# aluo7/ViT-SOM

Measured on AMD Instinct MI355X. Metric: images/sec/node ViT-SOM 40x40 CIFAR-10 bs512 (training step: fwd+bwd+all-reduce+AdamW), higher is better.
Workload: dtype f32 (Linear GEMMs on bf16 MFMA: forward from an exact 3xbf16 operand split, six products; weight / input gradients from a 2xbf16 split, three products, rel. error 4e-6)

## Files before the change

### include/vitsom_hip.h

```cpp
#ifndef VITSOM_HIP_H
#define VITSOM_HIP_H

#include <stddef.h>
#include <stdint.h>

#ifdef __cplusplus
extern "C" {
#endif

typedef struct ihipStream_t* vsom_stream_t;

#define VSOM_OK 0
#define VSOM_EINVAL (-1)
#define VSOM_EALIGN (-2)
#define VSOM_EUNSUPPORTED (-3)
#define VSOM_EWORKSPACE (-4)

#define VSOM_VERSION 100

#define VSOM_DIST_COSINE 0
#define VSOM_DIST_EUCLIDEAN 1
#define VSOM_DIST_MANHATTAN 2

int vsom_version(void);
const char* vsom_last_error_string(void);

int vsom_linear_fwd(const float* X, long ldx, const float* W, const float* bias, float* Y, long ldy,
                    int M, int N, int K, vsom_stream_t stream);

int vsom_linear_gelu_fwd(const float* X, long ldx, const float* W, const float* bias, float* Ygrad,
                         float* Yact, int M, int N, int K, vsom_stream_t stream);

int vsom_linear_relu_fwd(const float* X, long ldx, const float* W, const float* bias, float* Ygrad,
                         float* Yact, int M, int N, int K, vsom_stream_t stream);

int vsom_linear_residual_fwd(const float* X, long ldx, const float* W, const float* bias,
                             const float* R, long ldr, int r_mod, float* Y, long ldy, int M, int N,
                             int K, vsom_stream_t stream);

int vsom_linear_bwd_input(const float* dY, long lddy, const float* W, float* dX, long lddx, int M,
                          int N, int K, int accumulate, const float* gelu_grad, vsom_stream_t stream);

int vsom_linear_bwd_input_t(const float* dY, long lddy, const float* Wt, float* dX, long lddx, int M,
                            int N, int K, int accumulate, const float* gelu_grad, vsom_stream_t stream);

int vsom_transpose_many(const float* src_base, float* dst_base, const long long* table, int count,
                        int max_rows, int max_cols, vsom_stream_t stream);

#define VSOM_GEMM_F32 0
#define VSOM_GEMM_SPLIT_BF16 1
#define VSOM_GEMM_SPLIT_BF16_GRAD3 2
int vsom_set_gemm_mode(int mode);
int vsom_get_gemm_mode(void);

size_t vsom_linear_bwd_weight_workspace_bytes(int M, int N, int K);
int vsom_linear_bwd_weight(const float* dY, long lddy, const float* X, long ldx, float* dW, float* db,
                           int M, int N, int K, void* ws, size_t ws_bytes, vsom_stream_t stream);

int vsom_patch_embed_fwd(const float* img, const float* Wpe, const float* bpe, const float* pos,
                         const float* cls_token, float* tokens, float* xp_ws, int B, int C, int S,
                         int p, int E, vsom_stream_t stream);
size_t vsom_patch_embed_bwd_workspace_bytes(int B, int C, int S, int p, int E);
int vsom_patch_embed_bwd(const float* dtokens, const float* xp_ws, float* dWpe, float* dbpe,
                         float* dcls_token, int B, int C, int S, int p, int E, void* ws,
                         size_t ws_bytes, vsom_stream_t stream);

int vsom_layernorm_fwd(const float* X, const float* gamma, const float* beta, float* Y, float* mean,
                       float* rstd, int rows, int cols, float eps, vsom_stream_t stream);
size_t vsom_layernorm_bwd_workspace_bytes(int rows, int cols);
int vsom_layernorm_bwd(const float* dY, const float* X, const float* mean, const float* rstd,
                       const float* gamma, const float* resid, float* dX, float* dgamma, float* dbeta,
                       int rows, int cols, void* ws, size_t ws_bytes, vsom_stream_t stream);
#define VSOM_LN_JOB_WORDS 4
int vsom_layernorm_bwd_deferrable(int rows, int cols);
int vsom_layernorm_bwd_partial(const float* dY, const float* X, const float* mean, const float* rstd,
                               const float* gamma, const float* resid, float* dX, int rows, int cols, void* part,
                               size_t part_bytes, vsom_stream_t stream);
int vsom_layernorm_bwd_finish_many(const int64_t* jobs_dev, int first, int count, int max_cols, vsom_stream_t stream);

int vsom_linear_bwd_input_ln_supported(int M, int N, int K);
size_t vsom_linear_bwd_input_ln_partial_bytes(int M, int K);
int vsom_linear_bwd_input_ln(const float* dY, long lddy, const float* Wt, int M, int N, int K, const float* X,
                             const float* mean, const float* rstd, const float* gamma, const float* resid, float* dX,
                             float* dgamma, float* dbeta, void* ws, size_t ws_bytes, vsom_stream_t stream);
int vsom_linear_bwd_input_ln_partial(const float* dY, long lddy, const float* Wt, int M, int N, int K, const float* X,
                                     const float* mean, const float* rstd, const float* gamma, const float* resid,
// ... 138 lines not shown
```

### vit_som_amd/_lib.py

```python
import ctypes as C
import os

import torch

_HERE = os.path.dirname(os.path.abspath(__file__))
LIB_PATH = os.path.join(_HERE, "libvitsom_hip.so")

c_fp = C.c_void_p
c_stream = C.c_void_p

SIGNATURES = {
    "vsom_version": (C.c_int, []),
    "vsom_last_error_string": (C.c_char_p, []),
    "vsom_linear_fwd": (C.c_int, [c_fp, C.c_long, c_fp, c_fp, c_fp, C.c_long, C.c_int, C.c_int, C.c_int, c_stream]),
    "vsom_linear_gelu_fwd": (C.c_int, [c_fp, C.c_long, c_fp, c_fp, c_fp, c_fp, C.c_int, C.c_int, C.c_int, c_stream]),
    "vsom_linear_relu_fwd": (C.c_int, [c_fp, C.c_long, c_fp, c_fp, c_fp, c_fp, C.c_int, C.c_int, C.c_int, c_stream]),
    "vsom_l1_loss_workspace_bytes": (C.c_size_t, [C.c_long]),
    "vsom_l1_loss": (C.c_int, [c_fp, c_fp, c_fp, c_fp, C.c_float, C.c_long, c_fp, C.c_size_t, c_stream]),
    "vsom_linear_residual_fwd": (C.c_int, [c_fp, C.c_long, c_fp, c_fp, c_fp, C.c_long, C.c_int, c_fp, C.c_long,
                                           C.c_int, C.c_int, C.c_int, c_stream]),
    "vsom_linear_bwd_input": (C.c_int, [c_fp, C.c_long, c_fp, c_fp, C.c_long, C.c_int, C.c_int, C.c_int, C.c_int,
                                        c_fp, c_stream]),
    "vsom_linear_bwd_input_t": (C.c_int, [c_fp, C.c_long, c_fp, c_fp, C.c_long, C.c_int, C.c_int, C.c_int, C.c_int,
                                          c_fp, c_stream]),
    "vsom_transpose_many": (C.c_int, [c_fp, c_fp, C.c_void_p, C.c_int, C.c_int, C.c_int, c_stream]),
    "vsom_set_gemm_mode": (C.c_int, [C.c_int]),
    "vsom_get_gemm_mode": (C.c_int, []),
    "vsom_linear_bwd_weight_workspace_bytes": (C.c_size_t, [C.c_int, C.c_int, C.c_int]),
    "vsom_linear_bwd_weight": (C.c_int, [c_fp, C.c_long, c_fp, C.c_long, c_fp, c_fp, C.c_int, C.c_int, C.c_int,
                                         c_fp, C.c_size_t, c_stream]),
    "vsom_patch_embed_fwd": (C.c_int, [c_fp, c_fp, c_fp, c_fp, c_fp, c_fp, c_fp, C.c_int, C.c_int, C.c_int, C.c_int,
                                       C.c_int, c_stream]),
    "vsom_patch_embed_bwd_workspace_bytes": (C.c_size_t, [C.c_int] * 5),
    "vsom_patch_embed_bwd": (C.c_int, [c_fp, c_fp, c_fp, c_fp, c_fp, C.c_int, C.c_int, C.c_int, C.c_int, C.c_int,
                                       c_fp, C.c_size_t, c_stream]),
    "vsom_layernorm_fwd": (C.c_int, [c_fp, c_fp, c_fp, c_fp, c_fp, c_fp, C.c_int, C.c_int, C.c_float, c_stream]),
    "vsom_layernorm_bwd_workspace_bytes": (C.c_size_t, [C.c_int, C.c_int]),
    "vsom_layernorm_bwd": (C.c_int, [c_fp] * 9 + [C.c_int, C.c_int, c_fp, C.c_size_t, c_stream]),
    "vsom_layernorm_bwd_deferrable": (C.c_int, [C.c_int, C.c_int]),
    "vsom_layernorm_bwd_partial": (C.c_int, [c_fp] * 7 + [C.c_int, C.c_int, c_fp, C.c_size_t, c_stream]),
    "vsom_layernorm_bwd_finish_many": (C.c_int, [c_fp, C.c_int, C.c_int, C.c_int, c_stream]),
    "vsom_linear_bwd_input_ln_supported": (C.c_int, [C.c_int, C.c_int, C.c_int]),
    "vsom_linear_bwd_input_ln_partial_bytes": (C.c_size_t, [C.c_int, C.c_int]),
    "vsom_linear_bwd_input_ln": (C.c_int, [c_fp, C.c_long, c_fp, C.c_int, C.c_int, C.c_int] + [c_fp] * 8 + [c_fp, C.c_size_t, c_stream]),
    "vsom_linear_bwd_input_ln_partial": (C.c_int, [c_fp, C.c_long, c_fp, C.c_int, C.c_int, C.c_int] + [c_fp] * 6 + [c_fp, C.c_size_t, c_stream]),
    "vsom_attention_fwd": (C.c_int, [c_fp, c_fp, c_fp, C.c_int, C.c_int, C.c_int, C.c_int, c_stream]),
    "vsom_attention_bwd": (C.c_int, [c_fp] * 6 + [C.c_int] * 4 + [c_stream]),
    "vsom_set_attention_fused": (C.c_int, [C.c_int]),
    "vsom_attention_probs": (C.c_int, [c_fp, c_fp, c_fp, C.c_int, C.c_int, C.c_int, C.c_int, c_stream]),
    "vsom_attention_q1_fwd": (C.c_int, [c_fp] * 4 + [C.c_int] * 4 + [c_stream]),
    "vsom_attention_q1_bwd": (C.c_int, [c_fp] * 7 + [C.c_int] * 4 + [c_stream]),
    "vsom_rows_add": (C.c_int, [c_fp, C.c_long, c_fp, C.c_long, C.c_int, C.c_int, c_stream]),
    "vsom_tape_begin": (C.c_int, []),
    "vsom_tape_cut": (C.c_int, []),
    "vsom_tape_pause": (C.c_int, [C.c_int]),
    "vsom_tape_end": (C.c_int, []),
    "vsom_tape_recording": (C.c_int, []),
    "vsom_tape_segment_ops": (C.c_int, [C.c_int, C.c_int]),
    "vsom_tape_replay": (C.c_int, [C.c_int, C.c_int]),
    "vsom_tape_destroy": (C.c_int, [C.c_int]),
# ... 170 lines not shown
```

### vit_som_amd/csrc/gemm_f32.hip

```cpp
#include "gemm_f32.h"
#include "gemm_x6.h"
#include "gemm_x6_tn.h"

#include <atomic>

#include <stdarg.h>
#include <stdlib.h>

namespace vsom {

static thread_local char g_err[512] = "no error";
void set_error(const char* fmt, ...) {
    va_list ap;
    va_start(ap, fmt);
    vsnprintf(g_err, sizeof(g_err), fmt, ap);
    va_end(ap);
}
const char* last_error() { return g_err; }

static std::atomic<int> g_gemm_mode{VSOM_GEMM_SPLIT_BF16_GRAD3};
int gemm_mode() { return g_gemm_mode.load(std::memory_order_relaxed); }
static bool split_engine() { return gemm_mode() != VSOM_GEMM_F32; }
int gemm_grad_products() { return gemm_mode() == VSOM_GEMM_SPLIT_BF16_GRAD3 ? 3 : 6; }

// ... 99 lines not shown
    return VSOM_EUNSUPPORTED;
}

template <int WAVES, int VEC>
__global__ __launch_bounds__(WAVES * 64) void reduce_slabs_kernel(const float* __restrict__ slabs, long stride,
                                                                  int nslabs, float* __restrict__ out1, long n1,
                                                                  float* __restrict__ out2, long off2, long n2,
                                                                  int nb1, int vec) {
    __shared__ __attribute__((aligned(16))) f32x4 sh[WAVES][64];
    reduce_slabs_body<WAVES, VEC>(sh, (int)blockIdx.x, slabs, stride, nslabs, out1, n1, out2, off2, n2, nb1, vec);
}

int reduce_slabs2_internal(const float* slabs, long stride, int nslabs, float* out1, long n1, float* out2, long off2,
                           long n2, hipStream_t stream) {
    if (n1 <= 0 && n2 <= 0) return VSOM_OK;
    if (!out2) n2 = 0;
    const int vec = aligned16(slabs) && (stride % 4 == 0) && (off2 % 4 == 0);
    if (n1 + n2 <= 4096 && nslabs >= 32) {
        const int nb1 = cdiv(n1, 64), nb2 = n2 > 0 ? cdiv(n2, 64) : 0;
        VSOM_LAUNCH((reduce_slabs_kernel<16, 1>), dim3(nb1 + nb2), dim3(1024), 0, stream, slabs, stride, nslabs, out1,
                           n1, out2, off2, n2, nb1, vec);
    } else {
        const int nb1 = cdiv(n1, 256), nb2 = n2 > 0 ? cdiv(n2, 256) : 0;
        VSOM_LAUNCH((reduce_slabs_kernel<4, 4>), dim3(nb1 + nb2), dim3(256), 0, stream, slabs, stride, nslabs, out1, n1,
                           out2, off2, n2, nb1, vec);
    }
    VSOM_LAUNCH_CHECK("reduce_slabs_kernel");
}

int reduce_slabs_internal(const float* slabs, long stride, int nslabs, float* out, long n, hipStream_t stream) {
    return reduce_slabs2_internal(slabs, stride, nslabs, out, n, nullptr, 0, 0, stream);
}

int choose_splits(int tiles, int ktiles, int max_splits, bool prefer_xcd_multiple) {
    static int slots = 0;
    if (!slots) {
        int dev = 0, cus = 256;
        if (hipGetDevice(&dev) == hipSuccess) {
            hipDeviceProp_t p;
            if (hipGetDeviceProperties(&p, dev) == hipSuccess && p.multiProcessorCount > 0) cus = p.multiProcessorCount;
        }
        slots = 3 * cus;
    }
    if (max_splits > ktiles) max_splits = ktiles;
    if (max_splits < 1) max_splits = 1;
    static const double eff[4] = {1.0, 0.64, 0.80, 1.0};
    const int per_cu = slots / 3;
    double best = 1e30;
    int best_s = 1;
    for (int s = 1; s <= max_splits; ++s) {
        const int per = cdiv(ktiles, s);
        if (cdiv(ktiles, per) != s) continue;
        const long blocks = (long)tiles * s;
        const long full = blocks / slots;
        const long rest = blocks - full * slots;
        const int share = (int)((rest + per_cu - 1) / per_cu);
        const double passes = 3.0 * full + (share ? share / eff[share] : 0.0);
        double cost = passes * (per + 3.5) + 0.003 * tiles * s;
        if (prefer_xcd_multiple && s % 8 == 0) cost *= 0.93;
        if (cost < best) { best = cost; best_s = s; }
    }
    return best_s;
}
struct TnPlan { int cfg; int splits; };
static TnPlan bwd_weight_plan(int M, int N, int K) {
    TnPlan p;
    p.cfg = (N % 192 == 0 && K % 64 == 0) ? 1 : (N % 96 == 0 && K % 96 == 0) ? 2 : 0;
    if (p.cfg == 0) {
        p.splits = choose_splits(cdiv(N, gemm_tile_m(false, false, N)) * cdiv(K, 64), cdiv(M, 32), 128);
        return p;
    }
    const int tiles = p.cfg == 1 ? (N / 192) * (K / 64) : (N / 96) * (K / 96);
    const int ktiles = cdiv(M, 32);
    int s = (384 + tiles / 2) / tiles;
    if (s > ktiles) s = ktiles;
    if (s < 1) s = 1;
    const int per = cdiv(ktiles, s);
    p.splits = cdiv(ktiles, per);
    return p;
}
static long pad4(long n) { return (n + 3) & ~3L; }

static bool ln_fused_width(int K) { return K == 192 || K == 96; }
static int ln_fused_tiles(int M, int K) { return cdiv(M, K == 192 ? 64 : 128); }

static int linear_bwd_input_ln_launch(const float* dY, long lddy, const float* Wt, int M, int N, int K, const float* X,
                                      const float* mean, const float* rstd, const float* gamma, const float* resid,
                                      float* dX, float* part, size_t part_bytes, hipStream_t stream) {
    VSOM_REQUIRE(dY && Wt && X && mean && rstd && gamma && dX, VSOM_EINVAL, "linear_bwd_input_ln: null pointer");
    VSOM_REQUIRE(M > 0 && N > 0 && lddy >= N, VSOM_EINVAL, "linear_bwd_input_ln: bad shape M=%d N=%d lddy=%ld", M, N, lddy);
    VSOM_REQUIRE(vsom_linear_bwd_input_ln_supported(M, N, K), VSOM_EUNSUPPORTED,
                 "linear_bwd_input_ln: unsupported (M=%d N=%d K=%d, gemm mode %d)", M, N, K, gemm_mode());
    VSOM_REQUIRE(aligned16(dY) && aligned16(Wt) && aligned16(X) && aligned16(gamma) && aligned16(dX) &&
                 (!resid || aligned16(resid)) && lddy % 4 == 0 && N % 4 == 0, VSOM_EALIGN,
                 "linear_bwd_input_ln: operands must be 16-byte aligned (lddy, N multiples of 4)");
    VSOM_REQUIRE(part && aligned16(part) && part_bytes >= vsom_linear_bwd_input_ln_partial_bytes(M, K), VSOM_EWORKSPACE,
                 "linear_bwd_input_ln: partial buffer too small or misaligned");
    const long ab = operand_bytes(M, lddy, N), bb = operand_bytes(K, N, N);
    VSOM_REQUIRE(ab < 0xFFFF0000L && (long)M * K * 4 < 0xFFFF0000L, VSOM_EUNSUPPORTED, "linear_bwd_input_ln: operand larger than 4 GB");
    GemmP g = {};
    g.A = dY; g.lda = lddy; g.B = Wt; g.ldb = N; g.C = dX; g.ldc = K;
    g.M = M; g.N = K; g.K = N; g.alpha = 1.f;
    g.ktiles_per_split = cdiv(N, 32);
    g.a_vec = g.b_vec = 1;
    g.a_bytes = (unsigned)ab; g.b_bytes = (unsigned)bb;
    g.products = gemm_grad_products();
    g.ln_x = X; g.ln_mean = mean; g.ln_rstd = rstd; g.ln_gamma = gamma; g.ln_resid = resid; g.ln_part = part;
    const dim3 grid(ln_fused_tiles(M, K)), block(256);
    const bool x3 = g.products == 3;
    if (K == 192) {
        if (x3) VSOM_LAUNCH((gemm_x6_ln_kernel<3, 2, 2, 2>), grid, block, 0, stream, g);
// ... 3 lines not shown
        else VSOM_LAUNCH((gemm_x6_ln_kernel<3, 4, 1, 3>), grid, block, 0, stream, g);
    }
    VSOM_LAUNCH_CHECK("gemm_x6_ln_kernel");
}


int linear_bwd_weight_impl(const float* dY, long lddy, const float* X, long ldx, float* dW, float* db, int M, int N,
                           int K, int a_seg, int a_stride, int a_off, void* ws, size_t ws_bytes,
                           hipStream_t stream) {
    VSOM_REQUIRE(dY && X && dW, VSOM_EINVAL, "linear_bwd_weight: null pointer");
    VSOM_REQUIRE(lddy >= N && ldx >= K, VSOM_EINVAL, "linear_bwd_weight: leading dimension too small");
    VSOM_REQUIRE(ws && ws_bytes >= vsom_linear_bwd_weight_workspace_bytes(M, N, K), VSOM_EWORKSPACE,
                 "linear_bwd_weight: workspace too small (%zu < %zu)", ws_bytes,
                 vsom_linear_bwd_weight_workspace_bytes(M, N, K));
    VSOM_REQUIRE(aligned16(ws), VSOM_EALIGN, "linear_bwd_weight: workspace must be 16-byte aligned");
    const TnPlan plan = bwd_weight_plan(M, N, K);
    const int splits = plan.splits;
    const long wlen = pad4((long)N * K), blen = pad4(N);
    float* slab = static_cast<float*>(ws);
    const long a_last = a_seg ? (long)((M - 1) / a_seg) * a_stride + a_off + (M - 1) % a_seg : M - 1;
    const long ab = (a_last * lddy + N) * 4, bb = ((long)(M - 1) * ldx + K) * 4;
    const bool tn_ok = plan.cfg != 0 && split_engine() && aligned16(dY) && aligned16(X) &&
                       lddy % 4 == 0 && ldx % 4 == 0 && ab < 0xFFFF0000L && bb < 0xFFFF0000L &&
                       (a_seg == 0 || (a_seg % 32 == 0 && M % a_seg == 0));
    if (tn_ok) {
        TnP t = {};
        t.dY = dY; t.X = X; t.ldy = lddy; t.ldx = ldx; t.T = M; t.NO = N; t.KI = K;
        t.ktiles_per_split = cdiv(cdiv(M, 32), splits);
        t.a_seg = a_seg; t.a_stride = a_stride; t.a_off = a_off;
        t.slab = slab; t.slab_stride = wlen + blen;
        t.slab_bias = db ? slab + wlen : nullptr; t.slab_bias_stride = wlen + blen;
        t.a_bytes = (unsigned)ab; t.b_bytes = (unsigned)bb;
        const bool x3 = gemm_grad_products() == 3;
        if (plan.cfg == 1) {
            if (x3) VSOM_LAUNCH((gemm_x6_tn_kernel<3, 1, 2, 2, 2>), dim3((N / 192) * (K / 64) * splits), dim3(256), 0, stream, t);
            else VSOM_LAUNCH((gemm_x6_tn_kernel<3, 1, 2, 2, 3>), dim3((N / 192) * (K / 64) * splits), dim3(256), 0, stream, t);
        } else {
            if (x3) VSOM_LAUNCH((gemm_x6_tn_kernel<3, 1, 1, 3, 2>), dim3((N / 96) * (K / 96) * splits), dim3(192), 0, stream, t);
            else VSOM_LAUNCH((gemm_x6_tn_kernel<3, 1, 1, 3, 3>), dim3((N / 96) * (K / 96) * splits), dim3(192), 0, stream, t);
        }
        const int rc = hip_status(hipGetLastError(), "gemm_x6_tn_kernel");
        if (rc) return rc;
        return reduce_slabs2_internal(slab, wlen + blen, splits, dW, (long)N * K, db, wlen, db ? N : 0, stream);
    }
    GemmP g = {};
    g.A = dY; g.lda = lddy; g.B = X; g.ldb = ldx;
    g.M = N; g.N = K; g.K = M;
    g.a_seg = a_seg; g.a_stride = a_stride; g.a_off = a_off;
    g.slab = slab; g.slab_stride = wlen + blen;
    g.slab_bias = db ? slab + wlen : nullptr; g.slab_bias_stride = wlen + blen;
    int rc = launch_gemm(false, false, EPI_SLAB, g, splits, stream);
    if (rc) return rc;
    const int used = cdiv(cdiv(M, 32), cdiv(cdiv(M, 32), splits));
    return reduce_slabs2_internal(slab, wlen + blen, used, dW, (long)N * K, db, wlen, db ? N : 0, stream);
}

}

using namespace vsom;

extern "C" {

int vsom_version(void) { return VSOM_VERSION; }
const char* vsom_last_error_string(void) { return vsom::last_error(); }

int vsom_reduce_slabs(const float* slabs, long stride, int nslabs, float* out, long n, vsom_stream_t stream) {
    VSOM_REQUIRE(slabs && out && nslabs > 0 && n >= 0, VSOM_EINVAL, "reduce_slabs: bad arguments");
// ... 76 lines not shown
    return M > 0 && N > 0 && split_engine() && ln_fused_width(K) && ln_fused_tiles(M, K) >= 32;
}

size_t vsom_linear_bwd_input_ln_partial_bytes(int M, int K) {
    if (M <= 0 || !ln_fused_width(K)) return 0;
    return (size_t)ln_fused_tiles(M, K) * 2 * (size_t)K * sizeof(float);
}

int vsom_linear_bwd_input_ln(const float* dY, long lddy, const float* Wt, int M, int N, int K, const float* X,
                             const float* mean, const float* rstd, const float* gamma, const float* resid, float* dX,
                             float* dgamma, float* dbeta, void* ws, size_t ws_bytes, vsom_stream_t stream) {
    VSOM_REQUIRE(dgamma && dbeta, VSOM_EINVAL, "linear_bwd_input_ln: null pointer");
    float* part = static_cast<float*>(ws);
    const int rc = linear_bwd_input_ln_launch(dY, lddy, Wt, M, N, K, X, mean, rstd, gamma, resid, dX, part, ws_bytes, stream);
    if (rc) return rc;
    return reduce_slabs2_internal(part, 2L * K, ln_fused_tiles(M, K), dgamma, K, dbeta, K, K, stream);
}

int vsom_linear_bwd_input_ln_partial(const float* dY, long lddy, const float* Wt, int M, int N, int K, const float* X,
                                     const float* mean, const float* rstd, const float* gamma, const float* resid,
                                     float* dX, void* part, size_t part_bytes, vsom_stream_t stream) {
    return linear_bwd_input_ln_launch(dY, lddy, Wt, M, N, K, X, mean, rstd, gamma, resid, dX, static_cast<float*>(part),
                                      part_bytes, stream);
}

int vsom_set_gemm_mode(int mode) {
    VSOM_REQUIRE(mode == VSOM_GEMM_F32 || mode == VSOM_GEMM_SPLIT_BF16 || mode == VSOM_GEMM_SPLIT_BF16_GRAD3, VSOM_EINVAL,
                 "set_gemm_mode: unknown mode %d", mode);
    g_gemm_mode.store(mode, std::memory_order_relaxed);
    return VSOM_OK;
}
int vsom_get_gemm_mode(void) { return gemm_mode(); }

size_t vsom_linear_bwd_weight_workspace_bytes(int M, int N, int K) {
    if (M <= 0 || N <= 0 || K <= 0) return 0;
    const int s = bwd_weight_plan(M, N, K).splits;
    return (size_t)s * (size_t)(pad4((long)N * K) + pad4(N)) * sizeof(float);
}

int vsom_linear_bwd_weight(const float* dY, long lddy, const float* X, long ldx, float* dW, float* db, int M,
                           int N, int K, void* ws, size_t ws_bytes, vsom_stream_t stream) {
    return linear_bwd_weight_impl(dY, lddy, X, ldx, dW, db, M, N, K, 0, 0, 0, ws, ws_bytes, stream);
}

}
```

### vit_som_amd/csrc/gemm_x6_tn.h

```cpp
#pragma once
#include "gemm_x6.h"

namespace vsom {

typedef __attribute__((ext_vector_type(4))) short s16x4;
typedef __attribute__((ext_vector_type(8))) short s16x8;

struct TnP {
    const float* dY; const float* X;
    long ldy, ldx;
    int T, NO, KI;
    int ktiles_per_split;
    int a_seg, a_stride, a_off;
    float* slab; long slab_stride;
    float* slab_bias; long slab_bias_stride;
    unsigned a_bytes, b_bytes;
};

constexpr int tn_stride(int C) { return ((C * 2 + 63) / 128) * 128 + 64; }

__device__ __forceinline__ s16x4 tn_trread(const char* p) {
    return __builtin_amdgcn_ds_read_tr16_b64_v4i16((__attribute__((address_space(3))) s16x4*)p);
}

template <int WM, int WN, int WAVES_M, int WAVES_N, int NPL>
__global__ __launch_bounds__(WAVES_M * WAVES_N * 64) void gemm_x6_tn_kernel(const TnP g) {
    constexpr int BM = WAVES_M * WM * 32, BN = WAVES_N * WN * 32, NT = WAVES_M * WAVES_N * 64;
    constexpr int SA = tn_stride(BM), SB = tn_stride(BN), PA = 32 * SA, PB = 32 * SB;
    constexpr int FA = (32 * BM / 4 + NT - 1) / NT, FB = (32 * BN / 4 + NT - 1) / NT;
    static_assert(NPL * (PA + PB) >= NT * FA * 16, "LDS too small for the bias partials");
    __shared__ __attribute__((aligned(16))) char lds[NPL * (PA + PB)];
    char* As = lds; char* Bs = lds + NPL * PA;
    const int t = threadIdx.x, lane = t & 63, wave = t >> 6;
    const int wm0 = (wave / WAVES_N) * WM * 32, wn0 = (wave % WAVES_N) * WN * 32;
    const int tiles_n = g.KI / BN, tiles_m = g.NO / BM, ntiles = tiles_m * tiles_n;
    const int lid = xcd_remap(blockIdx.x, gridDim.x);
    const int z = lid / ntiles, rem = lid - z * ntiles;
    const int bm0 = (rem / tiles_n) * BM, bn0 = (rem % tiles_n) * BN;
    const int ktiles = (g.T + 31) >> 5;
    const int kt_begin = z * g.ktiles_per_split;
    int kt_end = kt_begin + g.ktiles_per_split;
    if (kt_end > ktiles) kt_end = ktiles;

    f32x16 acc[WM][WN];
#pragma unroll
    for (int i = 0; i < WM; ++i)
#pragma unroll
        for (int j = 0; j < WN; ++j)
#pragma unroll
            for (int v = 0; v < 16; ++v) acc[i][j][v] = 0.f;

    const __amdgpu_buffer_rsrc_t rsA = __builtin_amdgcn_make_buffer_rsrc(const_cast<float*>(g.dY), 0, (int)g.a_bytes, 0x00020000);
    const __amdgpu_buffer_rsrc_t rsB = __builtin_amdgcn_make_buffer_rsrc(const_cast<float*>(g.X), 0, (int)g.b_bytes, 0x00020000);
    f32x4 sa[FA], sb[FB];
    unsigned ga[FA], gb[FB];
    int la[FA], lb[FB];
#pragma unroll
    for (int i = 0; i < FA; ++i) {
        const int idx = i * NT + t, row = idx / (BM / 4), c4 = idx % (BM / 4);
        const bool ok = idx < 32 * BM / 4;
        ga[i] = ok ? (unsigned)(((long)row * g.ldy + bm0 + c4 * 4) * 4) : OOB;
        la[i] = ok ? row * SA + c4 * 8 : -1;
    }
#pragma unroll
    for (int i = 0; i < FB; ++i) {
        const int idx = i * NT + t, row = idx / (BN / 4), c4 = idx % (BN / 4);
        const bool ok = idx < 32 * BN / 4;
        gb[i] = ok ? (unsigned)(((long)row * g.ldx + bn0 + c4 * 4) * 4) : OOB;
        lb[i] = ok ? row * SB + c4 * 8 : -1;
    }
    const bool want_colsum = g.slab_bias != nullptr && bn0 == 0;
    f32x4 cs[FA];
#pragma unroll
    for (int i = 0; i < FA; ++i) cs[i] = f32x4{0.f, 0.f, 0.f, 0.f};

    auto gload = [&](int kt) {
        const long t0 = (long)kt << 5;
        const long ra = g.a_seg ? (t0 / g.a_seg) * g.a_stride + g.a_off + t0 % g.a_seg : t0;
        const unsigned sa_off = (unsigned)(ra * g.ldy * 4), sb_off = (unsigned)(t0 * g.ldx * 4);
#pragma unroll
        for (int i = 0; i < FA; ++i) sa[i] = __builtin_bit_cast(f32x4, __builtin_amdgcn_raw_buffer_load_b128(rsA, ga[i], sa_off, 0));
#pragma unroll
        for (int i = 0; i < FB; ++i) sb[i] = __builtin_bit_cast(f32x4, __builtin_amdgcn_raw_buffer_load_b128(rsB, gb[i], sb_off, 0));
    };
    auto lstore = [&]() {
#pragma unroll
        for (int i = 0; i < FA; ++i) {
            if (la[i] < 0) continue;
            if (want_colsum) cs[i] += sa[i];
            uint2 p1, p2, p3;
            if constexpr (NPL == 3) x6_split(sa[i], p1, p2, p3); else x3_split(sa[i], p1, p2);
            *reinterpret_cast<uint2*>(As + la[i]) = p1;
            *reinterpret_cast<uint2*>(As + PA + la[i]) = p2;
            if constexpr (NPL == 3) *reinterpret_cast<uint2*>(As + 2 * PA + la[i]) = p3;
        }
#pragma unroll
        for (int i = 0; i < FB; ++i) {
            if (lb[i] < 0) continue;
            uint2 p1, p2, p3;
            if constexpr (NPL == 3) x6_split(sb[i], p1, p2, p3); else x3_split(sb[i], p1, p2);
            *reinterpret_cast<uint2*>(Bs + lb[i]) = p1;
            *reinterpret_cast<uint2*>(Bs + PB + lb[i]) = p2;
            if constexpr (NPL == 3) *reinterpret_cast<uint2*>(Bs + 2 * PB + lb[i]) = p3;
        }
    };
    const int G = lane >> 4, q = (lane >> 2) & 3, pp = lane & 3;
    const int trow = 8 * (G >> 1) + q, tcol = 16 * (G & 1) + 4 * pp;
    int fa[WM], fbo[WN];
#pragma unroll
    for (int i = 0; i < WM; ++i) fa[i] = trow * SA + (wm0 + i * 32 + tcol) * 2;
#pragma unroll
    for (int j = 0; j < WN; ++j) fbo[j] = trow * SB + (wn0 + j * 32 + tcol) * 2;
    auto frag = [&](const char* base, int off, int stride, int ks) -> bf16x8 {
        const s16x4 lo = tn_trread(base + off + (ks * 16) * stride);
        const s16x4 hi = tn_trread(base + off + (ks * 16 + 4) * stride);
        const s16x8 v = {lo[0], lo[1], lo[2], lo[3], hi[0], hi[1], hi[2], hi[3]};
        return __builtin_bit_cast(bf16x8, v);
    };
    auto mfma_tile = [&]() {
#pragma unroll
        for (int ks = 0; ks < 2; ++ks) {
            bf16x8 a[WM][NPL], b[WN][NPL];
#pragma unroll
            for (int i = 0; i < WM; ++i)
#pragma unroll
                for (int pl = 0; pl < NPL; ++pl) a[i][pl] = frag(As + pl * PA, fa[i], SA, ks);
#pragma unroll
            for (int j = 0; j < WN; ++j)
#pragma unroll
                for (int pl = 0; pl < NPL; ++pl) b[j][pl] = frag(Bs + pl * PB, fbo[j], SB, ks);
#pragma unroll
            for (int i = 0; i < WM; ++i)
#pragma unroll
                for (int j = 0; j < WN; ++j) {
                    f32x16 c = acc[i][j];
                    if constexpr (NPL == 3) {
                        c = __builtin_amdgcn_mfma_f32_32x32x16_bf16(a[i][2], b[j][0], c, 0, 0, 0);
                        c = __builtin_amdgcn_mfma_f32_32x32x16_bf16(a[i][0], b[j][2], c, 0, 0, 0);
                        c = __builtin_amdgcn_mfma_f32_32x32x16_bf16(a[i][1], b[j][1], c, 0, 0, 0);
                    }
                    c = __builtin_amdgcn_mfma_f32_32x32x16_bf16(a[i][1], b[j][0], c, 0, 0, 0);
                    c = __builtin_amdgcn_mfma_f32_32x32x16_bf16(a[i][0], b[j][1], c, 0, 0, 0);
                    c = __builtin_amdgcn_mfma_f32_32x32x16_bf16(a[i][0], b[j][0], c, 0, 0, 0);
                    acc[i][j] = c;
                }
        }
    };
    if (kt_begin < kt_end) {
        gload(kt_begin);
        lstore();
    }
    __syncthreads();
    for (int kt = kt_begin; kt + 1 < kt_end; ++kt) {
        gload(kt + 1);
        __builtin_amdgcn_sched_barrier(0);
        mfma_tile();
        __builtin_amdgcn_sched_barrier(0);
        __syncthreads();
        lstore();
        __syncthreads();
    }
    if (kt_begin < kt_end) mfma_tile();

    if (want_colsum) {
        __syncthreads();
        f32x4* park = reinterpret_cast<f32x4*>(lds);
#pragma unroll
        for (int i = 0; i < FA; ++i) park[i * NT + t] = cs[i];
        __syncthreads();
        if (t < BM) {
            const int c4 = t >> 2, e = t & 3;
            float s = 0.f;
#pragma unroll 8
            for (int row = 0; row < 32; ++row) s += reinterpret_cast<const float*>(&park[row * (BM / 4) + c4])[e];
            g.slab_bias[(long)z * g.slab_bias_stride + bm0 + t] = s;
        }
    }
    const int r = lane & 31, h = lane >> 5;
    float* sl = g.slab + (long)z * g.slab_stride;
#pragma unroll
    for (int i = 0; i < WM; ++i)
#pragma unroll
        for (int j = 0; j < WN; ++j) {
            float* d = sl + (long)(bm0 + wm0 + i * 32 + 4 * h) * g.KI + bn0 + wn0 + j * 32 + r;
#pragma unroll
            for (int v = 0; v < 16; ++v) {
                *d = acc[i][j][v];
                d += (((v & 3) == 3) ? 5 : 1) * (long)g.KI;
            }
        }
}

}
```

### vit_som_amd/ops.py

```python
from typing import Optional

import torch

from . import _lib as _lib_mod
from ._lib import check, lib, ptr, stream

_scratch = {}
_retired = []

_timers = {}


def enable_timer(name: str):
    _timers[name] = []


def disable_timers():
    _timers.clear()


def timer_ms(name: str):
    ev = _timers.get(name, [])
    if not ev:
        return None
# ... 94 lines not shown
    return dx


def linear_bwd_input_t(dy, Wt, dx, accumulate=False, gelu_grad=None):
    M, N = dy.shape
    K = Wt.shape[0]
    _f32(dy, "dy"); _f32(Wt, "Wt"); _f32(dx, "dx")
    assert Wt.shape[1] == N and Wt.is_contiguous() and dx.shape == (M, K)
    if gelu_grad is not None:
        assert gelu_grad.is_contiguous() and gelu_grad.shape == (M, K)
    check(lib.vsom_linear_bwd_input_t(ptr(dy), _rows(dy), ptr(Wt), ptr(dx), _rows(dx), M, N, K, int(accumulate),
                                      ptr(gelu_grad), stream()), "vsom_linear_bwd_input_t")
    return dx


def transpose_many(src_base, dst_base, table, max_rows, max_cols):
    _f32(src_base, "src_base"); _f32(dst_base, "dst_base")
    assert table.dtype == torch.int64 and table.is_contiguous() and table.ndim == 2 and table.shape[1] == 4
    assert table.device == src_base.device == dst_base.device
    check(lib.vsom_transpose_many(ptr(src_base), ptr(dst_base), table.data_ptr(), table.shape[0], int(max_rows),
                                  int(max_cols), stream()), "vsom_transpose_many")
    return dst_base


GEMM_F32, GEMM_SPLIT_BF16, GEMM_SPLIT_BF16_GRAD3 = 0, 1, 2


def set_gemm_mode(mode: int):
    check(lib.vsom_set_gemm_mode(int(mode)), "vsom_set_gemm_mode")


def get_gemm_mode() -> int:
    return int(lib.vsom_get_gemm_mode())


def linear_bwd_weight(dy, x, dW, db):
    M, N = dy.shape
    K = x.shape[1]
    _f32(dy, "dy"); _f32(x, "x"); _f32(dW, "dW")
    assert x.shape[0] == M and dW.is_contiguous() and dW.numel() == N * K
    nbytes = lib.vsom_linear_bwd_weight_workspace_bytes(M, N, K)
    ws = scratch(nbytes, dy.device)
    check(lib.vsom_linear_bwd_weight(ptr(dy), _rows(dy), ptr(x), _rows(x), ptr(dW), ptr(db), M, N, K, ptr(ws), ws.numel(),
                                     stream()), "vsom_linear_bwd_weight")
    return dW, db


def patch_embed_fwd(img, Wpe, bpe, pos, cls_token, tokens, xp_ws, p):
    B, Cc, S, _ = img.shape
    E = Wpe.shape[0]
    for n_, t in (("img", img), ("Wpe", Wpe), ("tokens", tokens), ("xp_ws", xp_ws)):
        _f32(t, n_)
        assert t.is_contiguous(), n_
    check(lib.vsom_patch_embed_fwd(ptr(img), ptr(Wpe), ptr(bpe), ptr(pos), ptr(cls_token), ptr(tokens), ptr(xp_ws), B, Cc, S,
                                   p, E, stream()), "vsom_patch_embed_fwd")
    return tokens


def patch_embed_bwd(dtokens, xp_ws, dWpe, dbpe, dcls, B, Cc, S, p, E):
    assert dtokens.is_contiguous() and xp_ws.is_contiguous()
    nbytes = lib.vsom_patch_embed_bwd_workspace_bytes(B, Cc, S, p, E)
    ws = scratch(nbytes, dtokens.device)
    check(lib.vsom_patch_embed_bwd(ptr(dtokens), ptr(xp_ws), ptr(dWpe), ptr(dbpe), ptr(dcls), B, Cc, S, p, E, ptr(ws),
                                   ws.numel(), stream()), "vsom_patch_embed_bwd")


# ... 555 lines not shown
```

### vit_som_amd/step.py

```python
import weakref
from typing import Optional

import torch

from . import ops
from ._lib import Event, on_stream, stream_wait_stream
from .arena import ParamArena
from .tuning import hooks


class _StepLoss(torch.autograd.Function):

    @staticmethod
    def forward(ctx, anchor, model, x, y, gamma_t, T):
        ctx.model = model
        out, ctx.run_backward = model._step(x, y, gamma_t, T)
        ctx.forward_id = model._forward_id
        return out.clone()

    @staticmethod
    def backward(ctx, gout):
        m = ctx.model
        if ctx.forward_id != m._forward_id or m._seeds_consumed:
            raise RuntimeError("ViTSOM: backward() called twice for one training_step (or after a later forward): the "
                               "step's buffers and gradient seeds are single-use; gradient accumulation is not supported")
        m._seeds_consumed = True
        ctx.run_backward(gout)
        m._expose_grads()
        return None, None, None, None, None, None


class _StepTape:

    @staticmethod
    def _key(m):
        return (ops.get_gemm_mode(), ops.get_attention_fused(), hooks.signature(), m.world_size, m._use_vsom_comm, ops.stream())

    @classmethod
    @torch.no_grad()
    def step(cls, m, x, y, gamma_t: float, T: float):
        if not (hooks.launch_tape and x.is_cuda and (m.world_size == 1 or m._use_vsom_comm) and ops.tape_recording() == 0):
            return _ArenaOwner._step(m, x, y, gamma_t, T)
        x = m.vit._check_input(x)
        a = m.vit._buffers_for(x.shape[0], x.device)
        if not hasattr(a, "x_in"):
            a.x_in = torch.empty(a.B, m.vit.in_chans, m.vit.img_size, m.vit.img_size, dtype=torch.float32, device=a.device)
            a.y_in = torch.zeros(a.B, dtype=torch.int64, device=a.device)
            a.gout_in = torch.ones(1, dtype=torch.float32, device=a.device)
            a.steps_seen = 0
        xs, ys = a.x_in.copy_(x), a.y_in
        if m.classification:
            ys.copy_(y.view(-1))
        tape = a.__dict__.get("tape")
        if tape is not None and not tape.valid(m, a):
            tape.close()
            tape = a.tape = None
        if hooks.adamw_planes and m.som_layer._planes_shape_ok(a.B):
            m.som_layer._w_planes()
        if tape is None:
            a.steps_seen += 1
            if a.steps_seen <= 2:
                return _ArenaOwner._step(m, xs, ys, gamma_t, T)
            tid = ops.tape_begin()
            try:
                total = m._forward_losses(xs, ys, gamma_t, T, want_grad=True)
                a.gout_in.fill_(1.0)
                m._scale_seeds(a.gout_in)
                ops.tape_cut()
                m._backward()
# ... 263 lines not shown
```

Measured before the change: 56910.

## Add wide double-buffered weight-gradient GEMM tile with CU-based split count

```diff
diff --git a/include/vitsom_hip.h b/include/vitsom_hip.h
--- a/include/vitsom_hip.h
+++ b/include/vitsom_hip.h
@@ -52,6 +52,7 @@
 #define VSOM_GEMM_SPLIT_BF16_GRAD3 2
 int vsom_set_gemm_mode(int mode);
 int vsom_get_gemm_mode(void);
+int vsom_set_wgrad_tiles(int mode);
 
 size_t vsom_linear_bwd_weight_workspace_bytes(int M, int N, int K);
 int vsom_linear_bwd_weight(const float* dY, long lddy, const float* X, long ldx, float* dW, float* db,
diff --git a/lab/gemm_x6_tn_pf2_candidate.h b/lab/gemm_x6_tn_pf2_candidate.h
--- /dev/null
+++ b/lab/gemm_x6_tn_pf2_candidate.h
@@ -0,0 +1,229 @@
+#pragma once
+#include "gemm_x6.h"
+
+namespace vsom {
+
+typedef __attribute__((ext_vector_type(4))) short s16x4;
+typedef __attribute__((ext_vector_type(8))) short s16x8;
+
+struct TnP {
+    const float* dY; const float* X;
+    long ldy, ldx;
+    int T, NO, KI;
+    int ktiles_per_split;
+    int a_seg, a_stride, a_off;
+    float* slab; long slab_stride;
+    float* slab_bias; long slab_bias_stride;
+    unsigned a_bytes, b_bytes;
+};
+
+constexpr int tn_stride(int C) { return ((C * 2 + 63) / 128) * 128 + 64; }
+
+__device__ __forceinline__ s16x4 tn_trread(const char* p) {
+    return __builtin_amdgcn_ds_read_tr16_b64_v4i16((__attribute__((address_space(3))) s16x4*)p);
+}
+
+template <int WM, int WN, int WAVES_M, int WAVES_N, int NPL, int PF = 1>
+__global__ __launch_bounds__(WAVES_M * WAVES_N * 64) void gemm_x6_tn_kernel(const TnP g) {
+    constexpr int BM = WAVES_M * WM * 32, BN = WAVES_N * WN * 32, NT = WAVES_M * WAVES_N * 64;
+    constexpr int SA = tn_stride(BM), SB = tn_stride(BN), PA = 32 * SA, PB = 32 * SB;
+    constexpr int FA = (32 * BM / 4 + NT - 1) / NT, FB = (32 * BN / 4 + NT - 1) / NT;
+    static_assert(NPL * (PA + PB) >= NT * FA * 16, "LDS too small for the bias partials");
+    static_assert(PF == 1 || PF == 2, "one or two k-tiles of loads in flight");
+    __shared__ __attribute__((aligned(16))) char lds[NPL * (PA + PB)];
+    char* As = lds; char* Bs = lds + NPL * PA;
+    const int t = threadIdx.x, lane = t & 63, wave = t >> 6;
+    const int wm0 = (wave / WAVES_N) * WM * 32, wn0 = (wave % WAVES_N) * WN * 32;
+    const int tiles_n = g.KI / BN, tiles_m = g.NO / BM, ntiles = tiles_m * tiles_n;
+    const int lid = xcd_remap(blockIdx.x, gridDim.x);
+    const int z = lid / ntiles, rem = lid - z * ntiles;
+    const int bm0 = (rem / tiles_n) * BM, bn0 = (rem % tiles_n) * BN;
+    const int ktiles = (g.T + 31) >> 5;
+    const int kt_begin = z * g.ktiles_per_split;
+    int kt_end = kt_begin + g.ktiles_per_split;
+    if (kt_end > ktiles) kt_end = ktiles;
+
+    f32x16 acc[WM][WN];
+#pragma unroll
+    for (int i = 0; i < WM; ++i)
+#pragma unroll
+        for (int j = 0; j < WN; ++j)
+#pragma unroll
+            for (int v = 0; v < 16; ++v) acc[i][j][v] = 0.f;
+
+    const __amdgpu_buffer_rsrc_t rsA = __builtin_amdgcn_make_buffer_rsrc(const_cast<float*>(g.dY), 0, (int)g.a_bytes, 0x00020000);
+    const __amdgpu_buffer_rsrc_t rsB = __builtin_amdgcn_make_buffer_rsrc(const_cast<float*>(g.X), 0, (int)g.b_bytes, 0x00020000);
+    f32x4 sa[FA], sb[FB], sa2[PF == 2 ? FA : 1], sb2[PF == 2 ? FB : 1];
+    unsigned ga[FA], gb[FB];
+    int la[FA], lb[FB];
+#pragma unroll
+    for (int i = 0; i < FA; ++i) {
+        const int idx = i * NT + t, row = idx / (BM / 4), c4 = idx % (BM / 4);
+        const bool ok = idx < 32 * BM / 4;
+        ga[i] = ok ? (unsigned)(((long)row * g.ldy + bm0 + c4 * 4) * 4) : OOB;
+        la[i] = ok ? row * SA + c4 * 8 : -1;
+    }
+#pragma unroll
+    for (int i = 0; i < FB; ++i) {
+        const int idx = i * NT + t, row = idx / (BN / 4), c4 = idx % (BN / 4);
+        const bool ok = idx < 32 * BN / 4;
+        gb[i] = ok ? (unsigned)(((long)row * g.ldx + bn0 + c4 * 4) * 4) : OOB;
+        lb[i] = ok ? row * SB + c4 * 8 : -1;
+    }
+    const bool want_colsum = g.slab_bias != nullptr && bn0 == 0;
+    f32x4 cs[FA];
+#pragma unroll
+    for (int i = 0; i < FA; ++i) cs[i] = f32x4{0.f, 0.f, 0.f, 0.f};
+
+    auto gload = [&](f32x4(&va)[FA], f32x4(&vb)[FB], int kt) {
+        const long t0 = (long)kt << 5;
+        const long ra = g.a_seg ? (t0 / g.a_seg) * g.a_stride + g.a_off + t0 % g.a_seg : t0;
+        const unsigned sa_off = (unsigned)(ra * g.ldy * 4), sb_off = (unsigned)(t0 * g.ldx * 4);
+#pragma unroll
+        for (int i = 0; i < FA; ++i) va[i] = __builtin_bit_cast(f32x4, __builtin_amdgcn_raw_buffer_load_b128(rsA, ga[i], sa_off, 0));
+#pragma unroll
+        for (int i = 0; i < FB; ++i) vb[i] = __builtin_bit_cast(f32x4, __builtin_amdgcn_raw_buffer_load_b128(rsB, gb[i], sb_off, 0));
+    };
+    auto lstore = [&](const f32x4(&va)[FA], const f32x4(&vb)[FB]) {
+#pragma unroll
+        for (int i = 0; i < FA; ++i) {
+            if (la[i] < 0) continue;
+            if (want_colsum) cs[i] += va[i];
+            uint2 p1, p2, p3;
+            if constexpr (NPL == 3) x6_split(va[i], p1, p2, p3); else x3_split(va[i], p1, p2);
+            *reinterpret_cast<uint2*>(As + la[i]) = p1;
+            *reinterpret_cast<uint2*>(As + PA + la[i]) = p2;
+            if constexpr (NPL == 3) *reinterpret_cast<uint2*>(As + 2 * PA + la[i]) = p3;
+        }
+#pragma unroll
+        for (int i = 0; i < FB; ++i) {
+            if (lb[i] < 0) continue;
+            uint2 p1, p2, p3;
+            if constexpr (NPL == 3) x6_split(vb[i], p1, p2, p3); else x3_split(vb[i], p1, p2);
+            *reinterpret_cast<uint2*>(Bs + lb[i]) = p1;
+            *reinterpret_cast<uint2*>(Bs + PB + lb[i]) = p2;
+            if constexpr (NPL == 3) *reinterpret_cast<uint2*>(Bs + 2 * PB + lb[i]) = p3;
+        }
+    };
+    const int G = lane >> 4, q = (lane >> 2) & 3, pp = lane & 3;
+    const int trow = 8 * (G >> 1) + q, tcol = 16 * (G & 1) + 4 * pp;
+    int fa[WM], fbo[WN];
+#pragma unroll
+    for (int i = 0; i < WM; ++i) fa[i] = trow * SA + (wm0 + i * 32 + tcol) * 2;
+#pragma unroll
+    for (int j = 0; j < WN; ++j) fbo[j] = trow * SB + (wn0 + j * 32 + tcol) * 2;
+    auto frag = [&](const char* base, int off, int stride, int ks) -> bf16x8 {
+        const s16x4 lo = tn_trread(base + off + (ks * 16) * stride);
+        const s16x4 hi = tn_trread(base + off + (ks * 16 + 4) * stride);
+        const s16x8 v = {lo[0], lo[1], lo[2], lo[3], hi[0], hi[1], hi[2], hi[3]};
+        return __builtin_bit_cast(bf16x8, v);
+    };
+    auto mfma_tile = [&]() {
+#pragma unroll
+        for (int ks = 0; ks < 2; ++ks) {
+            bf16x8 a[WM][NPL], b[WN][NPL];
+#pragma unroll
+            for (int i = 0; i < WM; ++i)
+#pragma unroll
+                for (int pl = 0; pl < NPL; ++pl) a[i][pl] = frag(As + pl * PA, fa[i], SA, ks);
+#pragma unroll
+            for (int j = 0; j < WN; ++j)
+#pragma unroll
+                for (int pl = 0; pl < NPL; ++pl) b[j][pl] = frag(Bs + pl * PB, fbo[j], SB, ks);
+#pragma unroll
+            for (int i = 0; i < WM; ++i)
+#pragma unroll
+                for (int j = 0; j < WN; ++j) {
+                    f32x16 c = acc[i][j];
+                    if constexpr (NPL == 3) {
+                        c = __builtin_amdgcn_mfma_f32_32x32x16_bf16(a[i][2], b[j][0], c, 0, 0, 0);
+                        c = __builtin_amdgcn_mfma_f32_32x32x16_bf16(a[i][0], b[j][2], c, 0, 0, 0);
+                        c = __builtin_amdgcn_mfma_f32_32x32x16_bf16(a[i][1], b[j][1], c, 0, 0, 0);
+                    }
+                    c = __builtin_amdgcn_mfma_f32_32x32x16_bf16(a[i][1], b[j][0], c, 0, 0, 0);
+                    c = __builtin_amdgcn_mfma_f32_32x32x16_bf16(a[i][0], b[j][1], c, 0, 0, 0);
+                    c = __builtin_amdgcn_mfma_f32_32x32x16_bf16(a[i][0], b[j][0], c, 0, 0, 0);
+                    acc[i][j] = c;
+                }
+        }
+    };
+    if constexpr (PF == 1) {
+        if (kt_begin < kt_end) {
+            gload(sa, sb, kt_begin);
+            lstore(sa, sb);
+        }
+        __syncthreads();
+        for (int kt = kt_begin; kt + 1 < kt_end; ++kt) {
+            gload(sa, sb, kt + 1);
+            __builtin_amdgcn_sched_barrier(0);
+            mfma_tile();
+            __builtin_amdgcn_sched_barrier(0);
+            __syncthreads();
+            lstore(sa, sb);
+            __syncthreads();
+        }
+        if (kt_begin < kt_end) mfma_tile();
+    } else {
+        const int kt_last = kt_end - 1;
+        if (kt_begin < kt_end) {
+            gload(sa, sb, kt_begin);
+            gload(sa2, sb2, kt_begin + 1 < kt_end ? kt_begin + 1 : kt_last);
+            lstore(sa, sb);
+        }
+        __syncthreads();
+        int kt = kt_begin;
+        for (; kt + 2 < kt_end; kt += 2) {
+            gload(sa, sb, kt + 2);
+            __builtin_amdgcn_sched_barrier(0);
+            mfma_tile();
+            __builtin_amdgcn_sched_barrier(0);
+            __syncthreads();
+            lstore(sa2, sb2);
+            __syncthreads();
+            gload(sa2, sb2, kt + 3 < kt_end ? kt + 3 : kt_last);
+            __builtin_amdgcn_sched_barrier(0);
+            mfma_tile();
+            __builtin_amdgcn_sched_barrier(0);
+            __syncthreads();
+            lstore(sa, sb);
+            __syncthreads();
+        }
+        if (kt + 1 < kt_end) {
+            mfma_tile();
+            __syncthreads();
+            lstore(sa2, sb2);
+            __syncthreads();
+        }
+        if (kt_begin < kt_end) mfma_tile();
+    }
+
+    if (want_colsum) {
+        __syncthreads();
+        f32x4* park = reinterpret_cast<f32x4*>(lds);
+#pragma unroll
+        for (int i = 0; i < FA; ++i) park[i * NT + t] = cs[i];
+        __syncthreads();
+        if (t < BM) {
+            const int c4 = t >> 2, e = t & 3;
+            float s = 0.f;
+#pragma unroll 8
+            for (int row = 0; row < 32; ++row) s += reinterpret_cast<const float*>(&park[row * (BM / 4) + c4])[e];
+            g.slab_bias[(long)z * g.slab_bias_stride + bm0 + t] = s;
+        }
+    }
+    const int r = lane & 31, h = lane >> 5;
+    float* sl = g.slab + (long)z * g.slab_stride;
+#pragma unroll
+    for (int i = 0; i < WM; ++i)
+#pragma unroll
+        for (int j = 0; j < WN; ++j) {
+            float* d = sl + (long)(bm0 + wm0 + i * 32 + 4 * h) * g.KI + bn0 + wn0 + j * 32 + r;
+#pragma unroll
+            for (int v = 0; v < 16; ++v) {
+                *d = acc[i][j][v];
+                d += (((v & 3) == 3) ? 5 : 1) * (long)g.KI;
+            }
+        }
+}
+
+}
diff --git a/vit_som_amd/_lib.py b/vit_som_amd/_lib.py
--- a/vit_som_amd/_lib.py
+++ b/vit_som_amd/_lib.py
@@ -26,6 +26,7 @@
     "vsom_transpose_many": (C.c_int, [c_fp, c_fp, C.c_void_p, C.c_int, C.c_int, C.c_int, c_stream]),
     "vsom_set_gemm_mode": (C.c_int, [C.c_int]),
     "vsom_get_gemm_mode": (C.c_int, []),
+    "vsom_set_wgrad_tiles": (C.c_int, [C.c_int]),
     "vsom_linear_bwd_weight_workspace_bytes": (C.c_size_t, [C.c_int, C.c_int, C.c_int]),
     "vsom_linear_bwd_weight": (C.c_int, [c_fp, C.c_long, c_fp, C.c_long, c_fp, c_fp, C.c_int, C.c_int, C.c_int,
                                          c_fp, C.c_size_t, c_stream]),
diff --git a/vit_som_amd/csrc/gemm_f32.hip b/vit_som_amd/csrc/gemm_f32.hip
--- a/vit_som_amd/csrc/gemm_f32.hip
+++ b/vit_som_amd/csrc/gemm_f32.hip
@@ -155,16 +155,20 @@
     return reduce_slabs2_internal(slabs, stride, nslabs, out, n, nullptr, 0, 0, stream);
 }
 
-int choose_splits(int tiles, int ktiles, int max_splits, bool prefer_xcd_multiple) {
-    static int slots = 0;
-    if (!slots) {
-        int dev = 0, cus = 256;
+static int device_cus() {
+    static int cus = 0;
+    if (!cus) {
+        int dev = 0, n = 256;
         if (hipGetDevice(&dev) == hipSuccess) {
             hipDeviceProp_t p;
-            if (hipGetDeviceProperties(&p, dev) == hipSuccess && p.multiProcessorCount > 0) cus = p.multiProcessorCount;
-        }
-        slots = 3 * cus;
-    }
+            if (hipGetDeviceProperties(&p, dev) == hipSuccess && p.multiProcessorCount > 0) n = p.multiProcessorCount;
+        }
+        cus = n;
+    }
+    return cus;
+}
+int choose_splits(int tiles, int ktiles, int max_splits, bool prefer_xcd_multiple) {
+    const int slots = 3 * device_cus();
     if (max_splits > ktiles) max_splits = ktiles;
     if (max_splits < 1) max_splits = 1;
     static const double eff[4] = {1.0, 0.64, 0.80, 1.0};
@@ -186,6 +190,13 @@
     return best_s;
 }
 struct TnPlan { int cfg; int splits; };
+static std::atomic<int> g_wgrad_tiles{2};
+static int splits_for(int tiles, int ktiles, int target) {
+    int s = (target + tiles / 2) / tiles;
+    if (s > ktiles) s = ktiles;
+    if (s < 1) s = 1;
+    return cdiv(ktiles, cdiv(ktiles, s));
+}
 static TnPlan bwd_weight_plan(int M, int N, int K) {
     TnPlan p;
     p.cfg = (N % 192 == 0 && K % 64 == 0) ? 1 : (N % 96 == 0 && K % 96 == 0) ? 2 : 0;
@@ -195,11 +206,12 @@
     }
     const int tiles = p.cfg == 1 ? (N / 192) * (K / 64) : (N / 96) * (K / 96);
     const int ktiles = cdiv(M, 32);
-    int s = (384 + tiles / 2) / tiles;
-    if (s > ktiles) s = ktiles;
-    if (s < 1) s = 1;
-    const int per = cdiv(ktiles, s);
-    p.splits = cdiv(ktiles, per);
+    p.splits = splits_for(tiles, ktiles, 384);
+    const int wide = g_wgrad_tiles.load(std::memory_order_relaxed);
+    if (wide && gemm_grad_products() == 3 && N % 192 == 0 && K % 192 == 0) {
+        p.cfg = 3;
+        if (wide == 2) p.splits = splits_for((N / 192) * (K / 192), ktiles, 3 * device_cus() / 4);
+    }
     return p;
 }
 static long pad4(long n) { return (n + 3) & ~3L; }
@@ -269,7 +281,9 @@
         t.slab_bias = db ? slab + wlen : nullptr; t.slab_bias_stride = wlen + blen;
         t.a_bytes = (unsigned)ab; t.b_bytes = (unsigned)bb;
         const bool x3 = gemm_grad_products() == 3;
-        if (plan.cfg == 1) {
+        if (plan.cfg == 3) {
+            VSOM_LAUNCH((gemm_x6_tn_kernel<3, 1, 2, 6, 2, 2>), dim3((N / 192) * (K / 192) * splits), dim3(768), 0, stream, t);
+        } else if (plan.cfg == 1) {
             if (x3) VSOM_LAUNCH((gemm_x6_tn_kernel<3, 1, 2, 2, 2>), dim3((N / 192) * (K / 64) * splits), dim3(256), 0, stream, t);
             else VSOM_LAUNCH((gemm_x6_tn_kernel<3, 1, 2, 2, 3>), dim3((N / 192) * (K / 64) * splits), dim3(256), 0, stream, t);
         } else {
@@ -412,6 +426,12 @@
 }
 int vsom_get_gemm_mode(void) { return gemm_mode(); }
 
+int vsom_set_wgrad_tiles(int mode) {
+    VSOM_REQUIRE(mode >= 0 && mode <= 2, VSOM_EINVAL, "set_wgrad_tiles: unknown mode %d", mode);
+    g_wgrad_tiles.store(mode, std::memory_order_relaxed);
+    return VSOM_OK;
+}
+
 size_t vsom_linear_bwd_weight_workspace_bytes(int M, int N, int K) {
     if (M <= 0 || N <= 0 || K <= 0) return 0;
     const int s = bwd_weight_plan(M, N, K).splits;
diff --git a/vit_som_amd/csrc/gemm_x6_tn.h b/vit_som_amd/csrc/gemm_x6_tn.h
--- a/vit_som_amd/csrc/gemm_x6_tn.h
+++ b/vit_som_amd/csrc/gemm_x6_tn.h
@@ -23,13 +23,15 @@
     return __builtin_amdgcn_ds_read_tr16_b64_v4i16((__attribute__((address_space(3))) s16x4*)p);
 }
 
-template <int WM, int WN, int WAVES_M, int WAVES_N, int NPL>
+template <int WM, int WN, int WAVES_M, int WAVES_N, int NPL, int STAGES = 1>
 __global__ __launch_bounds__(WAVES_M * WAVES_N * 64) void gemm_x6_tn_kernel(const TnP g) {
     constexpr int BM = WAVES_M * WM * 32, BN = WAVES_N * WN * 32, NT = WAVES_M * WAVES_N * 64;
     constexpr int SA = tn_stride(BM), SB = tn_stride(BN), PA = 32 * SA, PB = 32 * SB;
     constexpr int FA = (32 * BM / 4 + NT - 1) / NT, FB = (32 * BN / 4 + NT - 1) / NT;
     static_assert(NPL * (PA + PB) >= NT * FA * 16, "LDS too small for the bias partials");
-    __shared__ __attribute__((aligned(16))) char lds[NPL * (PA + PB)];
+    static_assert(STAGES == 1 || STAGES == 2, "one or two LDS stages");
+    constexpr int ST = NPL * (PA + PB);
+    __shared__ __attribute__((aligned(16))) char lds[STAGES * ST];
     char* As = lds; char* Bs = lds + NPL * PA;
     const int t = threadIdx.x, lane = t & 63, wave = t >> 6;
     const int wm0 = (wave / WAVES_N) * WM * 32, wn0 = (wave % WAVES_N) * WN * 32;
@@ -83,25 +85,25 @@
 #pragma unroll
         for (int i = 0; i < FB; ++i) sb[i] = __builtin_bit_cast(f32x4, __builtin_amdgcn_raw_buffer_load_b128(rsB, gb[i], sb_off, 0));
     };
-    auto lstore = [&]() {
+    auto lstore = [&](int so) {
 #pragma unroll
         for (int i = 0; i < FA; ++i) {
             if (la[i] < 0) continue;
             if (want_colsum) cs[i] += sa[i];
             uint2 p1, p2, p3;
             if constexpr (NPL == 3) x6_split(sa[i], p1, p2, p3); else x3_split(sa[i], p1, p2);
-            *reinterpret_cast<uint2*>(As + la[i]) = p1;
-            *reinterpret_cast<uint2*>(As + PA + la[i]) = p2;
-            if constexpr (NPL == 3) *reinterpret_cast<uint2*>(As + 2 * PA + la[i]) = p3;
+            *reinterpret_cast<uint2*>(As + so + la[i]) = p1;
+            *reinterpret_cast<uint2*>(As + so + PA + la[i]) = p2;
+            if constexpr (NPL == 3) *reinterpret_cast<uint2*>(As + so + 2 * PA + la[i]) = p3;
         }
 #pragma unroll
         for (int i = 0; i < FB; ++i) {
             if (lb[i] < 0) continue;
             uint2 p1, p2, p3;
             if constexpr (NPL == 3) x6_split(sb[i], p1, p2, p3); else x3_split(sb[i], p1, p2);
-            *reinterpret_cast<uint2*>(Bs + lb[i]) = p1;
-            *reinterpret_cast<uint2*>(Bs + PB + lb[i]) = p2;
-            if constexpr (NPL == 3) *reinterpret_cast<uint2*>(Bs + 2 * PB + lb[i]) = p3;
+            *reinterpret_cast<uint2*>(Bs + so + lb[i]) = p1;
+            *reinterpret_cast<uint2*>(Bs + so + PB + lb[i]) = p2;
+            if constexpr (NPL == 3) *reinterpret_cast<uint2*>(Bs + so + 2 * PB + lb[i]) = p3;
         }
     };
     const int G = lane >> 4, q = (lane >> 2) & 3, pp = lane & 3;
@@ -117,18 +119,18 @@
         const s16x8 v = {lo[0], lo[1], lo[2], lo[3], hi[0], hi[1], hi[2], hi[3]};
         return __builtin_bit_cast(bf16x8, v);
     };
-    auto mfma_tile = [&]() {
+    auto mfma_tile = [&](int so) {
 #pragma unroll
         for (int ks = 0; ks < 2; ++ks) {
             bf16x8 a[WM][NPL], b[WN][NPL];
 #pragma unroll
             for (int i = 0; i < WM; ++i)
 #pragma unroll
-                for (int pl = 0; pl < NPL; ++pl) a[i][pl] = frag(As + pl * PA, fa[i], SA, ks);
+                for (int pl = 0; pl < NPL; ++pl) a[i][pl] = frag(As + so + pl * PA, fa[i], SA, ks);
 #pragma unroll
             for (int j = 0; j < WN; ++j)
 #pragma unroll
-                for (int pl = 0; pl < NPL; ++pl) b[j][pl] = frag(Bs + pl * PB, fbo[j], SB, ks);
+                for (int pl = 0; pl < NPL; ++pl) b[j][pl] = frag(Bs + so + pl * PB, fbo[j], SB, ks);
 #pragma unroll
             for (int i = 0; i < WM; ++i)
 #pragma unroll
@@ -146,21 +148,41 @@
                 }
         }
     };
-    if (kt_begin < kt_end) {
-        gload(kt_begin);
-        lstore();
-    }
-    __syncthreads();
-    for (int kt = kt_begin; kt + 1 < kt_end; ++kt) {
-        gload(kt + 1);
-        __builtin_amdgcn_sched_barrier(0);
-        mfma_tile();
-        __builtin_amdgcn_sched_barrier(0);
-        __syncthreads();
-        lstore();
-        __syncthreads();
-    }
-    if (kt_begin < kt_end) mfma_tile();
+    if constexpr (STAGES == 1) {
+        if (kt_begin < kt_end) {
+            gload(kt_begin);
+            lstore(0);
+        }
+        __syncthreads();
+        for (int kt = kt_begin; kt + 1 < kt_end; ++kt) {
+            gload(kt + 1);
+            __builtin_amdgcn_sched_barrier(0);
+            mfma_tile(0);
+            __builtin_amdgcn_sched_barrier(0);
+            __syncthreads();
+            lstore(0);
+            __syncthreads();
+        }
+        if (kt_begin < kt_end) mfma_tile(0);
+    } else {
+        if (kt_begin < kt_end) {
+            gload(kt_begin);
+            lstore(0);
+            if (kt_begin + 1 < kt_end) gload(kt_begin + 1);
+        }
+        __syncthreads();
+        int so = 0;
+        for (int kt = kt_begin; kt + 1 < kt_end; ++kt) {
+            lstore(ST - so);
+            gload(kt + 2 < kt_end ? kt + 2 : kt + 1);
+            __builtin_amdgcn_sched_barrier(0);
+            mfma_tile(so);
+            __builtin_amdgcn_sched_barrier(0);
+            __syncthreads();
+            so = ST - so;
+        }
+        if (kt_begin < kt_end) mfma_tile(so);
+    }
 
     if (want_colsum) {
         __syncthreads();
diff --git a/vit_som_amd/ops.py b/vit_som_amd/ops.py
--- a/vit_som_amd/ops.py
+++ b/vit_som_amd/ops.py
@@ -150,6 +150,19 @@
 
 def get_gemm_mode() -> int:
     return int(lib.vsom_get_gemm_mode())
+
+
+def set_wgrad_tiles(mode):
+    global _wgrad_tiles
+    check(lib.vsom_set_wgrad_tiles(int(mode)), "vsom_set_wgrad_tiles")
+    _wgrad_tiles = int(mode)
+
+
+_wgrad_tiles = 2
+
+
+def get_wgrad_tiles() -> int:
+    return _wgrad_tiles
 
 
 def linear_bwd_weight(dy, x, dW, db):
diff --git a/vit_som_amd/step.py b/vit_som_amd/step.py
--- a/vit_som_amd/step.py
+++ b/vit_som_amd/step.py
@@ -34,7 +34,7 @@
 
     @staticmethod
     def _key(m):
-        return (ops.get_gemm_mode(), ops.get_attention_fused(), hooks.signature(), m.world_size, m._use_vsom_comm, ops.stream())
+        return (ops.get_gemm_mode(), ops.get_attention_fused(), ops.get_wgrad_tiles(), hooks.signature(), m.world_size, m._use_vsom_comm, ops.stream())
 
     @classmethod
     @torch.no_grad()
```

Result: faster. 58600, median of 6 (+3.0%).
